# UCL/gp_emulator

Hardware: NVIDIA B200
Metric: test-point predictions/sec (mean+var+grad, M=250, D=10, FP64) (higher is better)
Workload: dtype f64

## Files before the change

gp_emulator_b200/csrc/gpemu.cu:

```cuda
#include <cuda_runtime.h>
#include <pthread.h>
#include <sched.h>
#include <stdarg.h>
#include <stdint.h>
#include <stdio.h>
#include <stdlib.h>
#include <string.h>

#include <algorithm>
#include <atomic>
#include <chrono>
#include <condition_variable>
#include <deque>
#include <cmath>
#include <mutex>
#include <string>
#include <thread>
#include <vector>

#include "../../include/gpemu.h"
#include "launch.h"
#include "predict_generic.cuh"
#include "gpe_math.cuh"
#include "host_common.h"
#include "host_stream.h"
#include "invert.h"

using namespace gpe;

namespace {

thread_local char g_err[512] = "";
std::atomic<int64_t> g_launches{0};
long long* g_trace = nullptr;

int fail(int code, const char* fmt, ...) {
    va_list ap;
    va_start(ap, fmt);
    vsnprintf(g_err, sizeof(g_err), fmt, ap);
    va_end(ap);
    return code;
}

#define CUDA_TRY(expr)                                                                                   \
    do {                                                                                                 \
        cudaError_t _e = (expr);                                                                         \
        if (_e != cudaSuccess)                                                                           \
            return fail(GPE_ERR_CUDA, "%s failed: %s (%s:%d)", #expr, cudaGetErrorString(_e), __FILE__, __LINE__); \
    } while (0)

constexpr uint32_t kSmemMax = 232448;
inline uint32_t align_up(uint32_t x, uint32_t a) { return (x + a - 1) / a * a; }

constexpr int kHessFusedMaxDp = 16;

struct FullPlan {
    bool valid = false;
    int cfg = 0, TN = 0, WC = 0, GH = 1, ctas_per_sm = 1;
    int Mp = 0, nt_act = 0, kblk = 0, kbps = 0, nit = 0, nstage = 0, JC = 0, nchunks = 0;
    uint32_t off_bar = 0, off_sqw = 0, off_ks = 0, off_bst = 0, off_xc = 0, off_ts = 0, off_pa = 0, off_vred = 0;
    uint32_t stage_bytes = 0, smem = 0, ts_bytes = 0;
    uint32_t off_hts = 0;
    int NC = 0, kbh = 0, nit_h = 0;
};

struct Tf32Plan {
    bool valid = false;
    int DP = 0, Mp = 0, nslab = 0;
    bool big = false;
    int pass_cols = 0;
    uint32_t off_bar = 0, off_tmem = 0, off_a = 0, off_b = 0, off_x = 0, off_out = 0, off_vred = 0, bstage_bytes = 0, smem = 0;
};

struct MeanPlan {
    int JC = 0, nchunks = 0;
    uint32_t off_xc = 0, off_ts = 0, off_out = 0, smem = 0, smem_hess = 0;
};

struct BankMeanPlan {
    bool valid = false;
    int G = 0, ngroups = 0, JC = 0, nchunks = 0;
    uint32_t off_x = 0, off_a = 0, off_w = 0, off_ts = 0, smem = 0;
};

}

struct gpe_model {
    int device = 0, M = 0, D = 0, DP = 0, sms = 0;
    const DpKernels* kern = nullptr;
    double b = 0;
    double sqrt_w[32];
    bool has_invQ = false;
    bool symmetric = false;
    FullPlan full;
    FullPlan full_small;
    MeanPlan mean;
    double* d_xchunks_full = nullptr;
    double* d_stiled = nullptr;
    double* d_ptiled = nullptr;
    bool large_valid = false;
    int large_Mp = 0, large_kblk = 0, large_nstage = 0;
    int64_t large_chunk = 0;
    double* d_kscratch = nullptr;
    cudaEvent_t scratch_free = nullptr;
    std::mutex scratch_mu;
    double centre[32];
    bool hess_fused_ok = false;
    double* d_xchunks_mean = nullptr;
    bool generic = false;
    double* d_gen_xs = nullptr;
    double* d_gen_alpha = nullptr;
    double* d_gen_sqw = nullptr;
    double* d_gen_mu = nullptr;
    Tf32Plan tf, tfx;
    float* d_xa_f32 = nullptr;
    uint32_t* d_bslabs = nullptr;
    uint32_t* d_bslabs_lo = nullptr;
    std::vector<double> h_inputs, h_invQt, h_invQ;
    double h_expx[33];
    std::mutex host_mu;
    Slot slots[3];
};

struct gpe_bank {
    int device = 0, E = 0, M = 0, D = 0, W = 0;
    std::vector<gpe_model*> models;
    MeanBankEntry* d_entries = nullptr;
    BankMeanPlan gplan[2];
    double* d_gx = nullptr;
    double* d_galpha[2] = {nullptr, nullptr};
    double* d_gw[2] = {nullptr, nullptr};
    double* d_basis = nullptr;
    int Wp = 0;
    std::mutex host_mu;
    Slot slots[3];
    double* d_aux = nullptr;
    size_t aux_cap = 0;
    cudaEvent_t aux_ready = nullptr;
    std::mutex cost_mu;
    double* cost_d = nullptr;
    size_t cost_cap = 0;
    cudaEvent_t cost_free = nullptr;
    std::mutex solve_mu;
    void* solve_d = nullptr;
    size_t solve_cap = 0;
    int* solve_count = nullptr;
    cudaEvent_t solve_ev = nullptr;
};

struct gpe_multi {
    std::vector<int> devices;
    std::vector<gpe_model*> models;
    std::vector<gpe_bank*> banks;
    std::mutex route_mu;
    bool routed = false;
    std::vector<Relay> relays;
    std::vector<double> link_gbs;
};

namespace {

BankMeanPlan plan_bank_mean(int E, int M, int D, int DP, bool grad) {
    BankMeanPlan g;
    long best = (long)E * (3 * D + 13);
    const int per_em = grad ? 2 * D + 12 : D + 11;
    for (int G = 2; G <= 10; ++G) {
        if (!bank_group_ok(DP, G, grad)) continue;
        const long cost = (long)((E + G - 1) / G) * (G * per_em + 2 * D);
        if (cost < best) { best = cost; g.G = G; }
    }
    if (const char* e = getenv(grad ? "GPE_BANK_G" : "GPE_BANK_G_MEAN"))
        if (bank_group_ok(DP, atoi(e), grad)) g.G = atoi(e);
    if (g.G == 0) return g;
    const int GP = (g.G + 1) & ~1;
    g.ngroups = (E + g.G - 1) / g.G;
    const int m4 = (M + 3) / 4 * 4;
    g.JC = std::min(m4, 256);
    g.nchunks = (M + g.JC - 1) / g.JC;
    uint32_t off = 0;
    g.off_x = off; off += align_up((uint32_t)g.JC * x_pitch(DP) * 8u, 16);
    g.off_a = off; off += align_up((uint32_t)g.JC * GP * 8u, 16);
    g.off_w = off; off += align_up(2u * g.G * DP * 8u, 16);
    g.off_ts = off; off += align_up((uint32_t)kBankTN * (uint32_t)std::max(D, g.G * (grad ? DP + 1 : 1)) * 8u, 16);
    g.smem = off;
    g.valid = true;
    return g;
}

FullPlan plan_full(int M, int D, int DP, int small_Mp = 0) {
    FullPlan f;
    const int m32 = (M + 31) / 32 * 32, m64 = (M + 63) / 64 * 64;
    const uint32_t smem_cap = kSmemMax - 2048;
    if (small_Mp > 0) {
        f.cfg = 2; f.TN = 16; f.WC = 8; f.GH = 4; f.Mp = small_Mp; f.nt_act = small_Mp / 64;
    } else if (m32 <= 256) {
        f.cfg = 0; f.TN = 64; f.WC = 4; f.GH = 1; f.Mp = m32; f.nt_act = m32 / 32;
    } else if (m64 <= 512) {
        f.cfg = 1; f.TN = 32; f.WC = 8; f.GH = 2; f.Mp = m64; f.nt_act = m64 / 64;
    } else if (m64 <= 1024) {
        f.cfg = 2; f.TN = 16; f.WC = 8; f.GH = 4; f.Mp = m64; f.nt_act = m64 / 64;
    } else {
        return f;
    }
    f.ctas_per_sm = 1;
    f.kblk = (M + 3) / 4;
    f.kbps = (f.cfg == 0) ? 2 : 1;
    f.nit = (f.kblk + f.kbps - 1) / f.kbps;
    f.stage_bytes = (uint32_t)f.kbps * f.Mp * 32u;

    uint32_t off = 0;
    f.off_bar = off; off += 192;
    f.off_sqw = off; off += 256;
    f.off_ks = off; off += (uint32_t)f.TN * (f.Mp + 4) * 8u;
    f.ts_bytes = align_up((uint32_t)f.TN * (D + 1) * 8u, 16);
    f.off_ts = off; off += 2 * f.ts_bytes;
    f.off_pa = off; off += (f.GH > 1) ? align_up((uint32_t)f.GH * f.TN * (D + 1) * 8u, 16) : 0;
    f.off_vred = off; off += (uint32_t)f.WC * f.TN * 8u;
    if (DP <= kHessFusedMaxDp) {
        f.off_hts = off; off += align_up((uint32_t)f.TN * D * 8u, 16);
        f.NC = (DP * (DP + 1) / 2 + 7) / 8 * 8;
        f.kbh = (int)(f.stage_bytes / ((uint32_t)f.NC * 32u));
        f.nit_h = f.kbh > 0 ? (f.kblk + f.kbh - 1) / f.kbh : 0;
    }
    off = align_up(off, 128);
    const uint32_t fixed = off;
    const int m4 = (M + 3) / 4 * 4;
    const uint32_t row = (uint32_t)(x_pitch(DP) + 1) * 8u;
    {
        const uint32_t avail = smem_cap - fixed;
        const uint32_t resident = (uint32_t)m4 * row;
        if (avail >= resident + 3 * f.stage_bytes) {
            f.JC = m4; f.nchunks = 1;
        } else {
            if (avail < 2 * f.stage_bytes + 64 * row) return f;
            const int jc_max = (int)((avail - 2 * f.stage_bytes) / row) / 4 * 4;
            f.JC = std::min(std::min(jc_max, 256), m4); f.nchunks = (M + f.JC - 1) / f.JC;
        }
        f.nstage = (int)std::min<uint32_t>(8, (avail - (uint32_t)f.JC * row) / f.stage_bytes);
        if (f.nstage < 2) return f;
    }
    f.off_bst = fixed;
    f.off_xc = fixed + (uint32_t)f.nstage * f.stage_bytes;
    f.smem = f.off_xc + (uint32_t)f.JC * row;
    f.valid = f.smem <= smem_cap;
    return f;
}

MeanPlan plan_mean(int M, int D, int DP) {
    MeanPlan m;
    const int m4 = (M + 3) / 4 * 4;
    m.JC = std::min(m4, 256);
    m.nchunks = (M + m.JC - 1) / m.JC;
    uint32_t off = 0;
    m.off_xc = off; off += align_up((uint32_t)m.JC * (x_pitch(DP) + 1) * 8u, 16);
    m.off_ts = off; off += align_up((uint32_t)kMeanTN * (D + 1) * 8u, 16);
    m.off_out = off;
    m.smem = off;
    m.smem_hess = off + (uint32_t)kMeanTN * D * 8u * (uint32_t)(DP <= 12 ? D : (DP <= 16 ? 4 : 2));
    return m;
}

uint32_t mean_extent(const MeanPlan& mp, int D, int DP, bool hess) {
    uint32_t ext = std::max(mp.off_xc + (uint32_t)mp.JC * (x_pitch(DP) + 1) * 8u, mp.off_ts + (uint32_t)kMeanTN * (D + 1) * 8u);
    if (hess) ext = std::max(ext, mp.off_out + (uint32_t)kMeanTN * D * 8u * (uint32_t)(DP <= 12 ? D : (DP <= 16 ? 4 : 2)));
    return ext;
}

template <typename T>
cudaError_t upload(T** d, const std::vector<T>& h) {
    const cudaError_t e = cudaMalloc((void**)d, h.size() * sizeof(T));
    return e == cudaSuccess ? cudaMemcpy(*d, h.data(), h.size() * sizeof(T), cudaMemcpyHostToDevice) : e;
}

std::vector<double> pack_xchunks(int M, int D, int DP, int JC, int nchunks, const double* inputs,
                                 const double* sqrt_w, const double* invQt, double b) {
    const int XP = x_pitch(DP);
    std::vector<double> buf((size_t)nchunks * JC * (XP + 1), 0.0);
    for (int j = 0; j < M; ++j) {
        const int c = j / JC, jl = j - c * JC;
        double* base = buf.data() + (size_t)c * JC * (XP + 1);
        for (int d = 0; d < D; ++d) base[(size_t)jl * XP + d] = sqrt_w[d] * inputs[(size_t)j * D + d];
        base[(size_t)JC * XP + jl] = b * invQt[j];
    }
    return buf;
}

int check_device(int device, int* sms) {
    int n = 0;
    cudaError_t e = cudaGetDeviceCount(&n);
    if (e != cudaSuccess || n == 0)
        return fail(GPE_ERR_NO_DEVICE, "no CUDA device available (%s); libgpemu has no CPU fallback",
                    e == cudaSuccess ? "device count 0" : cudaGetErrorString(e));
    if (device < 0 || device >= n) return fail(GPE_ERR_INVALID, "device %d out of range [0, %d)", device, n);
    cudaDeviceProp prop;
    CUDA_TRY(cudaGetDeviceProperties(&prop, device));
    if (prop.major != 10)
        return fail(GPE_ERR_NO_DEVICE, "device %d is sm_%d%d; libgpemu kernels are built for sm_100a only", device,
                    prop.major, prop.minor);
    *sms = prop.multiProcessorCount;
    return GPE_OK;
}

constexpr double kHessFusedMaxR2 = 2000.0;

cudaError_t build_hessian_operand(gpe_model* m, const double* inputs, const double* invQt) {
    const FullPlan& f = m->full;
    const int M = m->M, D = m->D;
    memset(m->centre, 0, sizeof(m->centre));
    m->hess_fused_ok = false;
    if (getenv("GPE_HESS_DIRECT") != nullptr) return cudaSuccess;
    if (!f.valid || f.kbh < 1 || f.NC > M || f.NC > f.Mp) return cudaSuccess;
    double r2max = 0.0;
    for (int d = 0; d < D; ++d) {
        double lo = inputs[d], hi = inputs[d];
        for (int j = 1; j < M; ++j) { lo = std::min(lo, inputs[(size_t)j * D + d]); hi = std::max(hi, inputs[(size_t)j * D + d]); }
        m->centre[d] = m->sqrt_w[d] * 0.5 * (lo + hi);
        const double r = m->sqrt_w[d] * 0.5 * (hi - lo);
        r2max = std::max(r2max, r * r);
    }
    if (!(r2max <= kHessFusedMaxR2)) return cudaSuccess;
    std::vector<double> pt((size_t)f.kblk * f.NC * 4, 0.0);
    std::vector<double> xp(D);
    for (int j = 0; j < M; ++j) {
        for (int d = 0; d < D; ++d) xp[d] = m->sqrt_w[d] * inputs[(size_t)j * D + d] - m->centre[d];
        const double ba = m->b * invQt[j];
        int col = 0;
        for (int d = 0; d < D; ++d)
            for (int e = d; e < D; ++e, ++col) pt[((size_t)(j >> 2) * f.NC + col) * 4 + (j & 3)] = ba * xp[d] * xp[e];
    }
    const cudaError_t e = upload(&m->d_ptiled, pt);
    m->hess_fused_ok = e == cudaSuccess;
    return e;
}

cudaError_t setup_large(gpe_model* m, const double* invQ) {
    const int M = m->M;
    m->large_Mp = (M + 63) / 64 * 64;
    m->large_kblk = m->large_Mp / 4;
    m->large_nstage = 6;
    m->large_chunk = 16 * (int64_t)m->sms * 4;
    const size_t scratch = (size_t)(m->large_chunk / 16) * m->large_kblk * 64 * 8;
    cudaError_t e = cudaMalloc((void**)&m->d_kscratch, scratch);
    if (e == cudaSuccess) e = cudaMemset(m->d_kscratch, 0, scratch);
    if (e == cudaSuccess) e = cudaEventCreateWithFlags(&m->scratch_free, cudaEventDisableTiming);
    if (e != cudaSuccess || !invQ || M > GPE_MAX_TRAIN) return e;
    const size_t Mp = (size_t)m->large_Mp;
    std::vector<double> st((size_t)m->large_kblk * Mp * 4, 0.0);
    for (int j = 0; j < M; ++j)
        for (int i = 0; i < M; ++i) st[((size_t)(i >> 2) * Mp + j) * 4 + (i & 3)] = invQ[(size_t)j * M + i];
    e = upload(&m->d_stiled, st);
    m->large_valid = e == cudaSuccess;
    return e;
}

cudaError_t var_large(const gpe_model* m, double* var, int64_t ld_var, int64_t n, cudaStream_t st) {
    VarLargeParams v;
    memset(&v, 0, sizeof(v));
    v.kstar = m->d_kscratch; v.s_tiled = m->d_stiled; v.var = var; v.ld_var = ld_var; v.N = n;
    v.Mp = m->large_Mp; v.kblk = m->large_kblk; v.npass = (m->large_Mp + kVlPass - 1) / kVlPass;
    v.nstage = m->large_nstage; v.b = m->b;
    const size_t smem = 128 + kVlWarps * kVlTN * 8 + (size_t)v.nstage * kVlStageBytes;
    return launch_var_large(v, (int)std::min<int64_t>((n + kVlTN - 1) / kVlTN, m->sms), smem, st);
}

int predict_generic(gpe_model* m, const double* testing, int64_t N, double* mu, double* var, double* deriv, double* hess,
                    int64_t ld_mu, int64_t ld_var, int64_t ld_deriv, int64_t ld_hess, cudaStream_t st) {
    if (var != nullptr && !m->has_invQ) return fail(GPE_ERR_INVALID, "variance requested but the model was created without invQ");
    if (var != nullptr && !m->large_valid)
        return fail(GPE_ERR_UNSUPPORTED, "variance contraction supports M <= %d (got M = %d)", GPE_MAX_TRAIN, m->M);
    const int D = m->D;
    const size_t smem_k = ((size_t)(kGenTN + kGenJC) * (D + 1) + 128) * 8;
    std::lock_guard<std::mutex> scratch_lock(m->scratch_mu);
    CUDA_TRY(cudaStreamWaitEvent(st, m->scratch_free, 0));
    for (int64_t n0 = 0; n0 < N; n0 += m->large_chunk) {
        const int64_t n = std::min(m->large_chunk, N - n0);
        GenericParams p;
        memset(&p, 0, sizeof(p));
        p.testing = testing + n0 * D; p.N = n;
        p.mu = mu ? mu + n0 * ld_mu : nullptr;
        p.deriv = deriv ? deriv + n0 * ld_deriv : nullptr;
        p.hess = hess ? hess + n0 * ld_hess : nullptr;
        p.ld_mu = ld_mu; p.ld_deriv = ld_deriv; p.ld_hess = ld_hess;
        p.xs = m->d_gen_xs; p.alpha = m->d_gen_alpha; p.sqw = m->d_gen_sqw;
        p.kstar = m->d_kscratch; p.mu_tmp = m->d_gen_mu;
        p.M = m->M; p.D = D; p.kblk = m->large_kblk;
        const int64_t tiles = (n + kGenTN - 1) / kGenTN;
        CUDA_TRY(launch_kernel(k_generic_kstar, (unsigned)std::min<int64_t>(tiles, (int64_t)m->sms * 4), kGenThreads, smem_k, st, p));
        if (deriv != nullptr)
            CUDA_TRY(launch_kernel(k_generic_grad, dim3((unsigned)std::min<int64_t>(tiles, (int64_t)m->sms * 8), (unsigned)std::min((D + 15) / 16, 16)),
                                   kGenThreads, 0, st, p));
        if (var != nullptr) CUDA_TRY(var_large(m, var + n0 * ld_var, ld_var, n, st));
        if (hess != nullptr) CUDA_TRY(launch_kernel(k_generic_hess, (unsigned)std::min<int64_t>(n, (int64_t)m->sms * 8), kGenThreads, 0, st, p));
    }
    CUDA_TRY(cudaEventRecord(m->scratch_free, st));
    return GPE_OK;
}

enum class Path { generic, large, tiny, fused, mean };
struct CallPlan {
    Path path;
    const FullPlan* full = nullptr;
    bool fuse_hess = false;
};

CallPlan plan_call(const gpe_model* m, int64_t call_N, bool var, bool hess) {
    CallPlan c;
    if (m->generic) { c.path = Path::generic; return c; }
    static const bool no_tiny = getenv("GPE_NO_TINY") != nullptr;
    static const int64_t env_max = getenv("GPE_TINY_MAX") ? atoll(getenv("GPE_TINY_MAX")) : -1;
    const int64_t tiny_max = env_max >= 0 ? env_max : kTinyTN * (int64_t)(2 * m->sms / kTinyCluster);
    const FullPlan& f = m->full;
    const bool tiny = m->has_invQ && !no_tiny && f.valid && f.cfg == 0 && f.nchunks == 1 && m->DP <= 16 && call_N <= tiny_max;
    c.path = tiny ? Path::tiny : f.valid ? Path::fused : m->large_valid ? Path::large : Path::mean;
    c.fuse_hess = hess && m->hess_fused_ok && !tiny && (var ? !m->symmetric : f.cfg == 0);
    const bool small = m->full_small.valid && !c.fuse_hess && call_N <= 3 * 16 * (int64_t)m->sms;
    c.full = small ? &m->full_small : &m->full;
    return c;
}

int predict_device(gpe_model* m, const double* testing, int64_t N, double* mu, double* var, double* deriv,
                   double* hess, int64_t ld_mu, int64_t ld_var, int64_t ld_deriv, int64_t ld_hess,
                   cudaStream_t st, int64_t call_N = -1) {
    if (call_N < 0) call_N = N;
    if (N == 0) return GPE_OK;
    const CallPlan c = plan_call(m, call_N, var != nullptr, hess != nullptr);
    if (c.path == Path::generic) return predict_generic(m, testing, N, mu, var, deriv, hess, ld_mu, ld_var, ld_deriv, ld_hess, st);
    bool mean_done = false;
    static const bool force_full = getenv("GPE_FORCE_FULL") != nullptr;
    if (var != nullptr && c.path == Path::large) {
        std::lock_guard<std::mutex> scratch_lock(m->scratch_mu);
        CUDA_TRY(cudaStreamWaitEvent(st, m->scratch_free, 0));
        for (int64_t n0 = 0; n0 < N; n0 += m->large_chunk) {
            const int64_t n = std::min(m->large_chunk, N - n0);
            MeanParams p;
            memset(&p, 0, sizeof(p));
            p.testing = testing + n0 * m->D; p.N = n;
            p.mu = mu ? mu + n0 * ld_mu : nullptr;
            p.deriv = deriv ? deriv + n0 * ld_deriv : nullptr;
            p.ld_mu = ld_mu; p.ld_deriv = ld_deriv;
            p.xchunks = m->d_xchunks_mean; p.M = m->M; p.D = m->D; p.JC = m->mean.JC; p.nchunks = m->mean.nchunks;
            p.off_xc = m->mean.off_xc; p.off_ts = m->mean.off_ts; p.off_out = m->mean.off_out;
            p.smem_need = mean_extent(m->mean, m->D, m->DP, false);
            p.kstar = m->d_kscratch; p.kblk = m->large_kblk;
            memcpy(p.sqrt_w, m->sqrt_w, sizeof(p.sqrt_w));
            const int64_t mtiles = (n + kMeanTN - 1) / kMeanTN;
            CUDA_TRY(m->kern->mean(false, p, dim3((unsigned)std::min<int64_t>(mtiles, (int64_t)m->sms * 12)), m->mean.smem, st));
            CUDA_TRY(var_large(m, var + n0 * ld_var, ld_var, n, st));
        }
        CUDA_TRY(cudaEventRecord(m->scratch_free, st));
        mean_done = true;
        var = nullptr;
    }
    if (var != nullptr && c.path == Path::tiny) {
        const FullPlan& f = m->full;
        TinyParams p;
        memset(&p, 0, sizeof(p));
        p.testing = testing; p.N = N; p.mu = mu; p.var = var; p.deriv = deriv;
        p.ld_mu = ld_mu; p.ld_var = ld_var; p.ld_deriv = ld_deriv;
        p.xchunks = m->d_xchunks_full; p.s_tiled = m->d_stiled;
        p.M = m->M; p.D = m->D; p.JC = f.JC; p.Mp = f.Mp; p.kblk = f.kblk; p.b = m->b;
        memcpy(p.sqrt_w, m->sqrt_w, sizeof(p.sqrt_w));
        const size_t work = std::max<size_t>({(size_t)f.JC * (x_pitch(m->DP) + 1) + (size_t)kTinyTN * m->D,
                                              (size_t)16 * 16 * (m->DP + 1), (size_t)8 * 16 * 32});
        const size_t smem = ((size_t)kTinyTN * (f.Mp + 4) + work) * 8;
        const int grid = (int)((N + kTinyTN - 1) / kTinyTN) * kTinyCluster;
        CUDA_TRY(m->kern->tiny(p, grid, smem, st));
        mean_done = true;
        var = nullptr;
    }
    if (var != nullptr || c.fuse_hess || (force_full && m->full.valid)) {
        if (var != nullptr && !m->has_invQ) return fail(GPE_ERR_INVALID, "variance requested but the model was created without invQ");
        if (!m->full.valid)
            return fail(GPE_ERR_UNSUPPORTED, "variance contraction supports M <= %d (got M = %d)", GPE_MAX_TRAIN, m->M);
        const FullPlan& f = *c.full;
        FullParams p;
        memset(&p, 0, sizeof(p));
        p.testing = testing; p.N = N; p.mu = mu; p.var = var; p.deriv = deriv;
        p.ld_mu = ld_mu; p.ld_var = ld_var; p.ld_deriv = ld_deriv;
        p.xchunks = m->d_xchunks_full; p.s_tiled = m->d_stiled;
        p.M = m->M; p.D = m->D; p.Mp = f.Mp; p.nt_act = f.nt_act; p.kblk = f.kblk;
        p.nit = f.nit; p.nstage = f.nstage; p.lag = (f.nstage >= 3) ? 2 : 1; p.symmetric = (m->symmetric && var != nullptr) ? 1 : 0;
        if (const char* e = getenv("GPE_RING_LAG")) p.lag = std::max(1, std::min(atoi(e), f.nstage - 1));
        p.skew = (f.cfg == 0 && f.nt_act == 8) ? 300 : 0;
        if (const char* e = getenv("GPE_SKEW")) p.skew = atoi(e);
        p.JC = f.JC; p.nchunks = f.nchunks; p.b = m->b;
        p.off_bar = f.off_bar; p.off_sqw = f.off_sqw; p.off_ks = f.off_ks; p.off_bst = f.off_bst;
        p.off_xc = f.off_xc; p.off_ts = f.off_ts; p.off_pa = f.off_pa; p.off_vred = f.off_vred;
        p.stage_bytes = f.stage_bytes; p.ts_bytes = f.ts_bytes;
        memcpy(p.sqrt_w, m->sqrt_w, sizeof(p.sqrt_w));
        p.trace = g_trace;
        if (c.fuse_hess) {
            p.hess = hess; p.ld_hess = ld_hess; p.p_tiled = m->d_ptiled; p.kbh = f.kbh; p.nit_h = f.nit_h; p.off_hts = f.off_hts;
            memcpy(p.centre, m->centre, sizeof(p.centre));
            hess = nullptr;
        }
        const int64_t ntiles = (N + f.TN - 1) / f.TN;
        const int grid = (int)std::min<int64_t>(ntiles, (int64_t)m->sms * f.ctas_per_sm);
        CUDA_TRY(m->kern->full(f.cfg, p, grid, f.smem, st));
        mean_done = true;
    }
    const bool need_mean = !mean_done && (mu != nullptr || deriv != nullptr);
    if (need_mean || hess != nullptr) {
        const bool do_hess = hess != nullptr;
        MeanParams p;
        memset(&p, 0, sizeof(p));
        p.testing = testing; p.N = N;
        p.mu = mean_done ? nullptr : mu;
        p.deriv = mean_done ? nullptr : deriv;
        p.hess = hess;
        p.ld_mu = ld_mu; p.ld_deriv = ld_deriv; p.ld_hess = ld_hess;
        p.xchunks = m->d_xchunks_mean; p.M = m->M; p.D = m->D; p.JC = m->mean.JC; p.nchunks = m->mean.nchunks;
        p.off_xc = m->mean.off_xc; p.off_ts = m->mean.off_ts; p.off_out = m->mean.off_out;
        p.smem_need = mean_extent(m->mean, m->D, m->DP, do_hess);
        memcpy(p.sqrt_w, m->sqrt_w, sizeof(p.sqrt_w));
        const int64_t ntiles = (N + kMeanTN - 1) / kMeanTN;
        static const int env_mult = getenv("GPE_MEAN_GRID") ? atoi(getenv("GPE_MEAN_GRID")) : 0;
        const int mult = env_mult > 0 ? env_mult : (do_hess ? 8 : 12);
        const int grid = (int)std::min<int64_t>(ntiles, (int64_t)m->sms * mult);
        const size_t smem = do_hess ? m->mean.smem_hess : m->mean.smem;
        CUDA_TRY(m->kern->mean(do_hess, p, dim3(grid), smem, st));
    }
    return GPE_OK;
}

struct DeviceRestore {
    int dev = -1;
    DeviceRestore() { if (cudaGetDevice(&dev) != cudaSuccess) { cudaGetLastError(); dev = -1; } }
    ~DeviceRestore() { if (dev >= 0) cudaSetDevice(dev); }
};

struct IoList {
    IoSpec v[kMaxIo];
    int n = 0;
    int add(const void* host, int64_t width) {
        if (n >= kMaxIo) return -1;
        v[n].host = const_cast<void*>(host);
        v[n].width = width;
        return n++;
    }
};

void bind_thread_near_device(int device) {
    char bdf[32];
    if (cudaDeviceGetPCIBusId(bdf, sizeof(bdf), device) != cudaSuccess) { cudaGetLastError(); return; }
    for (char* c = bdf; *c; ++c) *c = (char)tolower(*c);
    const std::string path = std::string("/sys/bus/pci/devices/") + bdf + "/local_cpulist";
    FILE* f = fopen(path.c_str(), "r");
    if (!f) return;
    char line[4096];
    cpu_set_t set;
    CPU_ZERO(&set);
    int count = 0;
    if (fgets(line, sizeof(line), f)) {
        char* save = nullptr;
        for (char* tok = strtok_r(line, ",\n", &save); tok; tok = strtok_r(nullptr, ",\n", &save)) {
            int a = 0, b = 0;
            if (sscanf(tok, "%d-%d", &a, &b) == 2) { for (int i = a; i <= b && i < CPU_SETSIZE; ++i) { CPU_SET(i, &set); ++count; } }
            else if (sscanf(tok, "%d", &a) == 1 && a < CPU_SETSIZE) { CPU_SET(a, &set); ++count; }
        }
    }
    fclose(f);
    if (count > 0) pthread_setaffinity_np(pthread_self(), sizeof(set), &set);
}

template <typename Fn>
int run_per_device(int G, const int* devices, Fn fn) {
    std::vector<int> rcs(G, GPE_OK);
    std::vector<std::string> msgs(G);
    std::vector<std::thread> th;
    for (int g = 0; g < G; ++g)
        th.emplace_back([&, g] {
            bind_thread_near_device(devices[g]);
            if (cudaSetDevice(devices[g]) != cudaSuccess) rcs[g] = fail(GPE_ERR_CUDA, "cudaSetDevice(%d) failed", devices[g]);
            else rcs[g] = fn(g);
            if (rcs[g]) msgs[g] = gpe_last_error();
        });
    for (auto& t : th) t.join();
    for (int g = 0; g < G; ++g)
        if (rcs[g]) return fail(rcs[g], "device %d: %s", devices[g], msgs[g].c_str());
    return GPE_OK;
}

template <typename... T>
int take_outputs(unsigned flags, T*&... outs) {
    unsigned bit = GPE_WANT_MU;
    bool missing = false, any = false;
    auto take = [&](auto*& o) {
        if (!(flags & bit)) o = nullptr;
        else if (!o) missing = true;
        any = any || o != nullptr;
        bit <<= 1;
    };
    (take(outs), ...);
    if (missing) return fail(GPE_ERR_INVALID, "an output flag is set but its array is NULL");
    if (!any) return fail(GPE_ERR_INVALID, "no output requested");
    return GPE_OK;
}

struct CallIo {
    IoList in, out;
    int idx[6] = {-1, -1, -1, -1, -1, -1};
    template <typename T>
    T* at(void* const* chunk, int k) const { return idx[k] >= 0 ? (T*)chunk[idx[k]] : nullptr; }
};

CallIo model_io(int64_t D, const void* testing, const void* mu, const void* var, const void* deriv, const void* hess) {
    CallIo io;
    io.in.add(testing, D);
    io.idx[0] = mu ? io.out.add(mu, 1) : -1;
    io.idx[1] = var ? io.out.add(var, 1) : -1;
    io.idx[2] = deriv ? io.out.add(deriv, D) : -1;
    io.idx[3] = hess ? io.out.add(hess, D * D) : -1;
    return io;
}

struct SharedCall {
    const StreamPlan* plan;
    ChunkSource* src;
    const Relay* relay;
};

StreamPlan stream_plan(const CallIo& io, int64_t N, size_t ES, int sms, int shared_by = 0) {
    return plan_stream(io.in.v, io.in.n, io.out.v, io.out.n, N, ES, 64 * (int64_t)sms, std::max(shared_by, 1), shared_by == 0);
}

template <typename Launch>
int stream_call(Slot* slots, int device, int sms, const CallIo& io, int64_t N, size_t ES, const SharedCall* shared,
                Launch launch) {
    const StreamPlan pl = shared ? *shared->plan : stream_plan(io, N, ES, sms);
    int rc = prepare_slots(slots, pl, io.in.v, io.in.n, io.out.v, io.out.n, ES);
    if (rc) return rc;
    std::atomic<int64_t> cursor{0};
    const ChunkSource src = shared ? *shared->src : ChunkSource{&cursor, N, pl.CH};
    return stream_host(slots, device, pl, src, ES, io.in.v, io.in.n, io.out.v, io.out.n, launch, shared ? shared->relay : nullptr);
// ... 1421 lines not shown
```

gp_emulator_b200/csrc/predict_full.cuh:

```cuda
#pragma once
#include <cuda_runtime.h>
#include <stdint.h>
#include <type_traits>
#include "gpe_math.cuh"
#include "gpe_ptx.cuh"

namespace gpe {

constexpr int kMaxD = 32;

struct FullParams {
    const double* testing;
    int64_t N;
    double* mu;
    double* var;
    double* deriv;
    int64_t ld_mu, ld_var, ld_deriv;
    const double* xchunks;
    const double* s_tiled;
    int M, D;
    int Mp;
    int nt_act;
    int kblk;
    int nit;
    int nstage;
    int lag;
    int JC;
    int symmetric;
    int skew;
    int nchunks;
    double b;
    uint32_t off_bar, off_sqw, off_ks, off_bst, off_xc, off_ts, off_pa, off_vred;
    uint32_t ts_bytes;
    uint32_t stage_bytes;
    double* hess;
    int64_t ld_hess;
    const double* p_tiled;
    int kbh;
    int nit_h;
    uint32_t off_hts;
    long long* trace;
    double sqrt_w[kMaxD];
    double centre[kMaxD];
};

template <int I, int N, typename F>
__device__ __forceinline__ void static_for_impl(F& f) {
    if constexpr (I < N) {
        f(std::integral_constant<int, I>{});
        static_for_impl<I + 1, N>(f);
    }
}
template <int N, typename F>
__device__ __forceinline__ void static_for(F f) {
    static_for_impl<0, N>(f);
}

template <int MT, int NT, int WR, int WC, int DP, int MINB, int KB, bool FULLNT, bool SYM, bool HESS>
__global__ void __launch_bounds__(WR * WC * 32, MINB) k_predict_full(const FullParams p) {
    constexpr int NW = WR * WC;
    constexpr int NTHR = NW * 32;
    constexpr int TN = WR * MT * 8;
    constexpr int NHI = TN / 8;
    constexpr int GH = NW / NHI;
    constexpr int TPR = NTHR / TN;
    constexpr int NV = DP + 1;
    constexpr int XP = x_pitch(DP);
    static_assert((NW & (NW - 1)) == 0, "warp count must be a power of two");
    static_assert(NHI * GH == NW && NHI >= 1 && GH >= 1, "TN must be 8 * (a divisor of the warp count)");
    static_assert(TPR >= 1 && TPR * TN == NTHR, "TN must divide the thread count");
    static_assert(DP % 2 == 0, "DP even (16-byte rows)");
    constexpr bool kLateChores = (MT >= 4);
    constexpr int NMT = TN / 8;
    constexpr int CG = (NW >= NMT) ? NW / NMT : 1;
    constexpr int NCT = (DP * (DP + 1) / 2 + 7) / 8;
    constexpr int NC = NCT * 8;
    constexpr int NTH = (NCT + CG - 1) / CG;
    static_assert(!HESS || (NW % NMT == 0 && NW >= NMT), "phase C needs the row tiles to divide the warps");
    static_assert(!(HESS && SYM), "the fused Hessian is built for the plain variance operand only");

    extern __shared__ __align__(128) unsigned char smem[];
    uint64_t* bar_full = reinterpret_cast<uint64_t*>(smem + p.off_bar);
    uint64_t* bar_empty = bar_full + 8;
    uint64_t* bar_x = bar_full + 16;
    uint64_t* bar_t = bar_full + 17;
    double* sqw_s = reinterpret_cast<double*>(smem + p.off_sqw);
    double* Ks = reinterpret_cast<double*>(smem + p.off_ks);
    unsigned char* Bst = smem + p.off_bst;
    double* Xc = reinterpret_cast<double*>(smem + p.off_xc);
    double* pa_s = reinterpret_cast<double*>(smem + p.off_pa);
    double* vred = reinterpret_cast<double*>(smem + p.off_vred);
    double* hts = reinterpret_cast<double*>(smem + p.off_hts);
    __shared__ int htab[HESS ? 256 : 1];
    __shared__ double cen_s[HESS ? kMaxD : 1];
    __shared__ double exp_tab[64];

    const int tid = threadIdx.x, warp = tid >> 5, lane = tid & 31;
    const int D = p.D, M = p.M, Mp = p.Mp;
    const int pitch = Mp + 4;
    const int nstage = p.nstage;
    const int lag = p.lag;
    const int DV = D + 1;

    const int64_t ntiles = (p.N + TN - 1) / TN;
    const bool want_var = (p.var != nullptr);
    const bool want_hess = HESS && (p.hess != nullptr);
    const int nit_b = want_var ? p.nit : 0;
    const int nit_tot = nit_b + (want_hess ? p.nit_h : 0);
    const bool ts_tma_ok = (reinterpret_cast<uintptr_t>(p.testing) & 15) == 0;
    const uint32_t ts_tile_bytes = (uint32_t)TN * D * 8u;

    {
        uint32_t ext = umax2(p.off_bar + 192u, p.off_sqw + 256u);
        ext = umax2(ext, p.off_ks + (uint32_t)TN * (uint32_t)pitch * 8u);
        ext = umax2(ext, p.off_ts + 2u * p.ts_bytes);
        ext = umax2(ext, umax2((uint32_t)TN * (uint32_t)DV * 8u, ts_tile_bytes) + p.off_ts + p.ts_bytes);
        if (GH > 1) ext = umax2(ext, p.off_pa + (uint32_t)GH * TN * (uint32_t)DV * 8u);
        ext = umax2(ext, p.off_vred + (uint32_t)WC * TN * 8u);
        if (want_hess) ext = umax2(ext, p.off_hts + (uint32_t)TN * (uint32_t)D * 8u);
        if (nit_tot > 0) ext = umax2(ext, p.off_bst + (uint32_t)nstage * p.stage_bytes);
        ext = umax2(ext, p.off_xc + (uint32_t)p.JC * (XP + 1) * 8u);
        smem_guard(ext);
    }
    if (tid == 0) {
        for (int s = 0; s < nstage; ++s) {
            mbar_init(&bar_full[s], 1);
            mbar_init(&bar_empty[s], NW);
        }
        mbar_init(bar_x, 1);
        mbar_init(&bar_t[0], 1);
        mbar_init(&bar_t[1], 1);
        fence_mbar_init();
    }
    if (tid < kMaxD) sqw_s[tid] = p.sqrt_w[tid];
    exp_tab_load(exp_tab, tid);
    if (HESS) {
        if (tid < kMaxD) cen_s[tid] = p.centre[tid];
        for (int e = tid; e < p.D * p.D; e += NTHR) {
            const int d1 = e / p.D, d2 = e - d1 * p.D;
            const int lo = min(d1, d2), hi = max(d1, d2);
            htab[e] = d1 | (d2 << 8) | ((lo * p.D - lo * (lo - 1) / 2 + hi - lo) << 16);
        }
    }
    for (int r = warp; r < TN; r += NW)
        for (int c = M + lane; c < pitch; c += 32) Ks[r * pitch + c] = 0.0;
    __syncthreads();

    int cs = 0;
    uint32_t cpar = 0;
    auto issue = [&](int stage, int it_local) {
        if (HESS && it_local >= nit_b) {
            const int kb0 = (it_local - nit_b) * p.kbh;
            const uint32_t bytes = (uint32_t)min(p.kbh, p.kblk - kb0) * (uint32_t)NC * 32u;
            mbar_arrive_expect_tx(&bar_full[stage], bytes);
            tma_bulk_g2s(Bst + (size_t)stage * p.stage_bytes, p.p_tiled + (size_t)kb0 * NC * 4, bytes, &bar_full[stage]);
            return;
        }
        const int kb0 = it_local * KB;
        const int nkb = min(KB, p.kblk - kb0);
        unsigned char* dst = Bst + (size_t)stage * p.stage_bytes;
        if (!SYM) {
            const uint32_t bytes = (uint32_t)nkb * (uint32_t)Mp * 32u;
            mbar_arrive_expect_tx(&bar_full[stage], bytes);
            tma_bulk_g2s(dst, p.s_tiled + (size_t)kb0 * Mp * 4, bytes, &bar_full[stage]);
        } else {
            uint32_t total = 0;
            for (int kk = 0; kk < nkb; ++kk) total += (uint32_t)(Mp - 8 * ((kb0 + kk) >> 1)) * 32u;
            mbar_arrive_expect_tx(&bar_full[stage], total);
            for (int kk = 0; kk < nkb; ++kk) {
                const int c0 = 8 * ((kb0 + kk) >> 1);
                tma_bulk_g2s(dst + ((size_t)kk * Mp + c0) * 32, p.s_tiled + ((size_t)(kb0 + kk) * Mp + c0) * 4,
                             (uint32_t)(Mp - c0) * 32u, &bar_full[stage]);
            }
        }
    };
    auto issue_burst = [&]() {
        const int burst = min(nstage, nit_tot);
        if (lane == 0) {
            for (int i = warp; i < burst; i += NW) {
                int s = cs + i;
                if (s >= nstage) s -= nstage;
                issue(s, i);
            }
        }
    };
    auto refill = [&](int it) {
        if (it >= lag && lane == 0 && warp == (it & (NW - 1)) && it - lag + nstage < nit_tot) {
            const int ps = (cs >= lag) ? cs - lag : cs - lag + nstage;
            const uint32_t ppar = (cs >= lag) ? cpar : (cpar ^ 1);
            mbar_wait(&bar_empty[ps], ppar);
            issue(ps, it - lag + nstage);
        }
    };
    uint32_t xpar = 0;
    bool x_resident = false;

    uint32_t tpar = 0;
    auto prefetch_rows = [&](int64_t tile, int buf) -> bool {
        const int64_t n0 = tile * TN;
        if (!ts_tma_ok || n0 + TN > p.N) return false;
        fence_proxy_async();
        mbar_arrive_expect_tx(&bar_t[buf], ts_tile_bytes);
        tma_bulk_g2s(smem + p.off_ts + (size_t)buf * p.ts_bytes, p.testing + n0 * D, ts_tile_bytes, &bar_t[buf]);
        return true;
    };
    auto rows_prefetched = [&](int64_t tile) { return ts_tma_ok && (tile * TN + TN <= p.N); };

    const int g_low = lane & 7, n_low = lane >> 3;
    const int n_hi = warp % NHI, g_hi = warp / NHI;
    const int n_a = n_hi * 8 + n_low, n_b = n_a + 4;
    const int wrow = warp / WC;
    const int wcol = (SYM && ((warp >> 2) & 1)) ? (((warp % WC) & ~3) | (3 - ((warp % WC) & 3))) : warp % WC;
    const int nt_act = FULLNT ? NT : p.nt_act;

    int buf = 0;
    if (tid == 0 && blockIdx.x < ntiles) prefetch_rows(blockIdx.x, 0);
    int trace_tile = 0;
    const bool tracing = p.trace != nullptr && blockIdx.x == 0 && tid == 0;
#define GPE_TRACE(k) do { if (tracing && trace_tile < 64) p.trace[trace_tile * 8 + (k)] = clock64(); } while (0)

    for (int64_t tile = blockIdx.x; tile < ntiles; tile += gridDim.x, buf ^= 1) {
        const int64_t n0 = tile * TN;
        const int npts = (int)min((int64_t)TN, p.N - n0);
        double* ts_s = reinterpret_cast<double*>(smem + p.off_ts + (size_t)buf * p.ts_bytes);
        GPE_TRACE(0);
        if (!kLateChores && nit_tot > 0) issue_burst();

        if (rows_prefetched(tile)) {
            mbar_wait(&bar_t[buf], (tpar >> buf) & 1u);
            tpar ^= 1u << buf;
        } else {
            for (int e = tid; e < TN * D; e += NTHR) {
                const int r = e / D;
                const int64_t src = (r < npts) ? (n0 * D + e) : ((p.N - 1) * D + (e - r * D));
                ts_s[e] = __ldg(p.testing + src);
            }
            __syncthreads();
        }
        constexpr bool kTwoPass = DP > 16;
        double tsa[kTwoPass ? 1 : DP], tsb[kTwoPass ? 1 : DP];
        if constexpr (!kTwoPass) {
#pragma unroll
            for (int d = 0; d < DP; ++d) {
                tsa[d] = (d < D) ? ts_s[n_a * D + d] * sqw_s[d] : 0.0;
                tsb[d] = (d < D) ? ts_s[n_b * D + d] * sqw_s[d] : 0.0;
            }
        }
        if constexpr (HESS) {
            if (want_hess && g_hi == 0) {
#pragma unroll
                for (int d = 0; d < DP; ++d)
                    if ((d & 7) == g_low && d < D) {
                        hts[n_a * D + d] = tsa[d] - cen_s[d];
                        hts[n_b * D + d] = tsb[d] - cen_s[d];
                    }
            }
        }
        if (!x_resident && tid == 0) {
            const uint32_t bytes = (uint32_t)p.JC * (XP + 1) * 8u;
            mbar_arrive_expect_tx(bar_x, bytes);
            tma_bulk_g2s(Xc, p.xchunks, bytes, bar_x);
        }
        __syncthreads();
        if (kLateChores && nit_tot > 0) issue_burst();
        {
            const int64_t next = tile + gridDim.x;
            if (tid == ((kLateChores && NW > 4) ? 32 * (NW - 1) : 0) && next < ntiles) prefetch_rows(next, buf ^ 1);
        }

        GPE_TRACE(1);
        double va[NV], vb[NV];
#pragma unroll
        for (int i = 0; i < NV; ++i) va[i] = vb[i] = 0.0;

        for (int c = 0; c < p.nchunks; ++c) {
            if (!x_resident) {
                if (c > 0 && tid == 0) {
                    const uint32_t bytes = (uint32_t)p.JC * (XP + 1) * 8u;
                    mbar_arrive_expect_tx(bar_x, bytes);
                    tma_bulk_g2s(Xc, p.xchunks + (size_t)c * p.JC * (XP + 1), bytes, bar_x);
                }
                mbar_wait(bar_x, xpar);
                xpar ^= 1;
                if (p.nchunks == 1) x_resident = true;
            }
            const int jn = min(p.JC, M - c * p.JC);
            const double* al = Xc + p.JC * XP;
            double* krow_a = Ks + n_a * pitch + c * p.JC;
            double* krow_b = krow_a + 4 * pitch;
            if constexpr (kTwoPass) {
                auto sweep = [&](int n_r, double (&v1)[NV]) {
                    double* krow = Ks + n_r * pitch + c * p.JC;
                    double ts1[DP];
#pragma unroll
                    for (int d = 0; d < DP; ++d) ts1[d] = (d < D) ? ts_s[n_r * D + d] * sqw_s[d] : 0.0;
                    for (int jl = 8 * g_hi + g_low; jl < jn; jl += 8 * GH) {
                        const double2* xr = reinterpret_cast<const double2*>(Xc + jl * XP);
                        double u[DP];
                        double r = 0.0;
#pragma unroll
                        for (int q = 0; q < DP / 2; ++q) {
                            const double2 x2 = xr[q];
                            u[2 * q] = x2.x - ts1[2 * q];
                            u[2 * q + 1] = x2.y - ts1[2 * q + 1];
                            r = fma(u[2 * q], u[2 * q], r);
                            r = fma(u[2 * q + 1], u[2 * q + 1], r);
                        }
                        const double k = exp_neg_tab(-0.5 * r, exp_tab);
                        krow[jl] = k;
                        const double cj = k * al[jl];
                        v1[0] += cj;
#pragma unroll
                        for (int d = 0; d < DP; ++d) v1[1 + d] = fma(cj, u[d], v1[1 + d]);
                    }
                };
                sweep(n_a, va);
                sweep(n_b, vb);
            } else {
            int jl = 8 * g_hi + g_low;
                if (jl < jn) {
                    double2 xn[DP / 2];
                    double aln;
                    {
                        const double2* xr = reinterpret_cast<const double2*>(Xc + jl * XP);
    #pragma unroll
                        for (int q = 0; q < DP / 2; ++q) xn[q] = xr[q];
                        aln = al[jl];
                    }
                    for (; jl < jn; jl += 8 * GH) {
                        double2 x[DP / 2];
    #pragma unroll
                        for (int q = 0; q < DP / 2; ++q) x[q] = xn[q];
                        const double alj = aln;
                        {
                            const int jnx = min(jl + 8 * GH, jn - 1);
                            const double2* xr = reinterpret_cast<const double2*>(Xc + jnx * XP);
    #pragma unroll
                            for (int q = 0; q < DP / 2; ++q) xn[q] = xr[q];
                            aln = al[jnx];
                        }
                        double ua[DP], ub[DP];
                        double ra = 0.0, rb = 0.0;
    #pragma unroll
                        for (int q = 0; q < DP / 2; ++q) {
                            const int d = 2 * q;
                            ua[d] = x[q].x - tsa[d];
                            ub[d] = x[q].x - tsb[d];
                            ua[d + 1] = x[q].y - tsa[d + 1];
                            ub[d + 1] = x[q].y - tsb[d + 1];
                            ra = fma(ua[d], ua[d], ra);
                            rb = fma(ub[d], ub[d], rb);
                            ra = fma(ua[d + 1], ua[d + 1], ra);
                            rb = fma(ub[d + 1], ub[d + 1], rb);
                        }
                        const double ka = exp_neg_tab(-0.5 * ra, exp_tab);
                        const double kb = exp_neg_tab(-0.5 * rb, exp_tab);
                        krow_a[jl] = ka;
                        krow_b[jl] = kb;
                        const double ca = ka * alj, cb = kb * alj;
                        va[0] += ca;
                        vb[0] += cb;
    #pragma unroll
                        for (int d = 0; d < DP; ++d) {
                            va[1 + d] = fma(ca, ua[d], va[1 + d]);
                            vb[1 + d] = fma(cb, ub[d], vb[1 + d]);
                        }
                    }
                }
            }
            if (!x_resident) __syncthreads();
        }

        GPE_TRACE(2);
        double* outs = ts_s;
        if constexpr (kTwoPass) __syncthreads();
        {
            RS<NV> rs;
            rs.run(va, vb, lane);
            double* dst = ((GH == 1) ? outs : pa_s + g_hi * TN * DV) + ((lane & 4) ? n_b : n_a) * DV;
            const int half_base = (lane & 2) ? RS<NV>::H2 : 0;
            const int base3 = (lane & 1) ? RS<NV>::H3 : 0;
#pragma unroll
            for (int i = 0; i < RS<NV>::H3; ++i) {
                const int i2 = base3 + i;
                const int idx = half_base + i2;
                if (i2 < RS<NV>::H2 && idx < DV) dst[idx] = rs.r3[i];
            }
            __syncthreads();
            if (GH > 1) {
                for (int e = tid; e < TN * DV; e += NTHR) {
                    double sum = 0.0;
                    for (int gh = 0; gh < GH; ++gh) sum += pa_s[gh * TN * DV + e];
                    outs[e] = sum;
                }
                __syncthreads();
            }
        }
        {
            const int r = tid / TPR, q = tid % TPR;
            if (r < npts) {
                if (p.mu != nullptr && q == 0) p.mu[(n0 + r) * p.ld_mu] = outs[r * DV];
                if (p.deriv != nullptr) {
                    for (int d = q; d < D; d += TPR) p.deriv[(n0 + r) * p.ld_deriv + d] = sqw_s[d] * outs[r * DV + 1 + d];
                }
            }
        }

        GPE_TRACE(3);
        if (want_var) {
            double acc[MT][NT][2];
#pragma unroll
            for (int i = 0; i < MT; ++i)
#pragma unroll
                for (int j = 0; j < NT; ++j) acc[i][j][0] = acc[i][j][1] = 0.0;

            const double* a_base = Ks + (wrow * MT * 8 + (lane >> 2)) * pitch + (lane & 3);
            const int b_off = (wcol * 8 + (lane >> 2)) * 4 + (lane & 3);

            auto ring_step = [&](auto jm_c, int it) {
                constexpr int JM = decltype(jm_c)::value;
                refill(it);
                const int kb0 = it * KB;
                double a[KB][MT];
#pragma unroll
                for (int kk = 0; kk < KB; ++kk)
#pragma unroll
                    for (int i = 0; i < MT; ++i) a[kk][i] = a_base[i * 8 * pitch + (kb0 + kk) * 4];
                mbar_wait(&bar_full[cs], cpar);
                const double* bs = reinterpret_cast<const double*>(Bst + (size_t)cs * p.stage_bytes) + b_off;
#pragma unroll
                for (int kk = 0; kk < KB; ++kk) {
                    if (KB == 1 || kb0 + kk < p.kblk) {
                        const double* bk = bs + kk * Mp * 4;
#pragma unroll
                        for (int j = JM; j < NT; ++j) {
                            if (!FULLNT && j >= nt_act) break;
                            const double bf = bk[j * (WC * 32)];
#pragma unroll
                            for (int i = 0; i < MT; ++i) dmma_m8n8k4(acc[i][j][0], acc[i][j][1], a[kk][i], bf);
                        }
                    }
                }
                __syncwarp();
                if (lane == 0) mbar_arrive(&bar_empty[cs]);
                if (++cs == nstage) { cs = 0; cpar ^= 1; }
            };
            if (p.skew > 0 && ((warp >> 2) & 1)) {
                const long long t0 = clock64();
                while (clock64() - t0 < p.skew) {}
            }
            if constexpr (!SYM) {
                for (int it = 0; it < nit_b; ++it) ring_step(std::integral_constant<int, 0>{}, it);
            } else {
                int it = 0;
                static_for<NT>([&](auto jm_c) {
                    constexpr int JM = decltype(jm_c)::value;
                    const int it_end = min(nit_b, (WC * JM + wcol + 1) * (2 / KB));
                    for (; it < it_end; ++it) ring_step(jm_c, it);
                });
                for (; it < nit_b; ++it) ring_step(std::integral_constant<int, NT>{}, it);
            }

            GPE_TRACE(4);
            double vs[MT];
#pragma unroll
            for (int i = 0; i < MT; ++i) vs[i] = 0.0;
            const int odd = (lane >> 2) & 1;
            const double* k_base = Ks + (wrow * MT * 8 + (lane >> 2)) * pitch + wcol * 8 + 2 * (lane & 3);
#pragma unroll
            for (int j = 0; j < NT; ++j) {
                if (FULLNT || j < nt_act) {
#pragma unroll
                    for (int i = 0; i < MT; ++i) {
                        const double* kp = k_base + i * 8 * pitch + j * (WC * 8);
                        if (kLateChores) {
                            const double k_first = kp[odd], k_second = kp[odd ^ 1];
                            vs[i] = fma(acc[i][j][0], odd ? k_second : k_first, vs[i]);
                            vs[i] = fma(acc[i][j][1], odd ? k_first : k_second, vs[i]);
                        } else {
                            const double2 kk = *reinterpret_cast<const double2*>(kp);
                            vs[i] = fma(acc[i][j][0], kk.x, vs[i]);
                            vs[i] = fma(acc[i][j][1], kk.y, vs[i]);
                        }
                    }
                }
            }
#pragma unroll
            for (int i = 0; i < MT; ++i) {
                vs[i] += __shfl_xor_sync(0xffffffffu, vs[i], 1);
                vs[i] += __shfl_xor_sync(0xffffffffu, vs[i], 2);
                if ((lane & 3) == 0) vred[wcol * TN + wrow * MT * 8 + i * 8 + (lane >> 2)] = vs[i];
            }
            __syncthreads();
            if (tid < npts) {
                double v = 0.0;
#pragma unroll
                for (int w = 0; w < WC; ++w) v += vred[w * TN + tid];
                p.var[(n0 + tid) * p.ld_var] = p.b - p.b * p.b * v;
            }
        }
        if (HESS && want_hess) {
            GPE_TRACE(5);
            const int mt = warp % NMT, cg = warp / NMT;
            double hacc[NTH][2];
#pragma unroll
            for (int j = 0; j < NTH; ++j) hacc[j][0] = hacc[j][1] = 0.0;
            const double* a_base = Ks + (mt * 8 + (lane >> 2)) * pitch + (lane & 3);
            const int b_off = (cg * 8 + (lane >> 2)) * 4 + (lane & 3);
            for (int it = nit_b; it < nit_tot; ++it) {
                refill(it);
                const int kb0 = (it - nit_b) * p.kbh;
                const int nkb = min(p.kbh, p.kblk - kb0);
                mbar_wait(&bar_full[cs], cpar);
                const double* bs = reinterpret_cast<const double*>(Bst + (size_t)cs * p.stage_bytes) + b_off;
                const double* ap = a_base + kb0 * 4;
#pragma unroll 3
                for (int kk = 0; kk < nkb; ++kk) {
                    const double a = ap[kk * 4];
                    const double* bk = bs + kk * (NC * 4);
#pragma unroll
                    for (int j = 0; j < NTH; ++j) {
                        if (NCT % CG != 0 && cg + CG * j >= NCT) break;
                        dmma_m8n8k4(hacc[j][0], hacc[j][1], a, bk[j * (CG * 32)]);
                    }
                }
                __syncwarp();
                if (lane == 0) mbar_arrive(&bar_empty[cs]);
                if (++cs == nstage) { cs = 0; cpar ^= 1; }
            }
            GPE_TRACE(6);
            __syncthreads();
#pragma unroll
            for (int j = 0; j < NTH; ++j) {
                if (cg + CG * j < NCT)
                    *reinterpret_cast<double2*>(Ks + (mt * 8 + (lane >> 2)) * pitch + (cg + CG * j) * 8 + 2 * (lane & 3)) =
                        make_double2(hacc[j][0], hacc[j][1]);
            }
            __syncthreads();
            constexpr int NE = (DP * DP + 31) / 32;
            const int DD = D * D;
            int o1[NE], o2[NE], oc[NE];
            double ow[NE], od[NE];
#pragma unroll
            for (int i = 0; i < NE; ++i) {
                const int e = min(lane + 32 * i, DD - 1);
                const int t = htab[e];
                o1[i] = t & 255; o2[i] = (t >> 8) & 255; oc[i] = t >> 16;
                ow[i] = sqw_s[o1[i]] * sqw_s[o2[i]];
                od[i] = (o1[i] == o2[i]) ? ow[i] : 0.0;
            }
#pragma unroll 2
            for (int r = warp; r < npts; r += NW) {
                const double* s2 = Ks + r * pitch;
                const double* tp = hts + r * D;
                const double* g = outs + r * DV + 1;
                const double s0 = outs[r * DV];
                double* dst = p.hess + (n0 + r) * p.ld_hess;
#pragma unroll
                for (int i = 0; i < NE; ++i) {
                    const double t1 = tp[o1[i]], t2 = tp[o2[i]];
                    double v = s2[oc[i]];
                    v = fma(-t1, g[o2[i]], v);
                    v = fma(-t2, fma(t1, s0, g[o1[i]]), v);
                    v = fma(v, ow[i], -od[i] * s0);
                    if (lane + 32 * i < DD) dst[lane + 32 * i] = v;
                }
            }
            GPE_TRACE(7);
        }
        __syncthreads();
        if (!(HESS && want_hess)) GPE_TRACE(5);
        ++trace_tile;
    }
}

#undef GPE_TRACE

}
```

Baseline: 219.4 million.

## Pack multiple triangular k-blocks per ring stage in symmetric variance path

In the symmetric variance path each ring stage used to carry one k-block unit with trailing columns skipped, so stages were partly empty. A host-computed schedule now packs several consecutive shrinking triangular units into one stage buffer. This cuts the number of ring iterations, mbarrier waits and refills. The cost is a per-unit sub-step loop that walks a variable packed offset, plus a 512-byte schedule array added to the kernel parameters.

```diff
diff --git a/gp_emulator_b200/csrc/gpemu.cu b/gp_emulator_b200/csrc/gpemu.cu
--- a/gp_emulator_b200/csrc/gpemu.cu
+++ b/gp_emulator_b200/csrc/gpemu.cu
@@ -62,6 +62,8 @@
     uint32_t stage_bytes = 0, smem = 0, ts_bytes = 0;
     uint32_t off_hts = 0;
     int NC = 0, kbh = 0, nit_h = 0;
+    int sym_nit = 0;
+    uint16_t sym_stage_end[kMaxSymStages];
 };
 
 struct Tf32Plan {
@@ -207,6 +209,7 @@
     f.kbps = (f.cfg == 0) ? 2 : 1;
     f.nit = (f.kblk + f.kbps - 1) / f.kbps;
     f.stage_bytes = (uint32_t)f.kbps * f.Mp * 32u;
+    f.sym_nit = sym_stage_schedule(f.kblk, f.kbps, f.Mp, f.stage_bytes, f.sym_stage_end);
 
     uint32_t off = 0;
     f.off_bar = off; off += 192;
@@ -480,6 +483,10 @@
         p.xchunks = m->d_xchunks_full; p.s_tiled = m->d_stiled;
         p.M = m->M; p.D = m->D; p.Mp = f.Mp; p.nt_act = f.nt_act; p.kblk = f.kblk;
         p.nit = f.nit; p.nstage = f.nstage; p.lag = (f.nstage >= 3) ? 2 : 1; p.symmetric = (m->symmetric && var != nullptr) ? 1 : 0;
+        if (p.symmetric) {
+            p.nit = f.sym_nit;
+            memcpy(p.sym_stage_end, f.sym_stage_end, sizeof(p.sym_stage_end));
+        }
         if (const char* e = getenv("GPE_RING_LAG")) p.lag = std::max(1, std::min(atoi(e), f.nstage - 1));
         p.skew = (f.cfg == 0 && f.nt_act == 8) ? 300 : 0;
         if (const char* e = getenv("GPE_SKEW")) p.skew = atoi(e);
diff --git a/gp_emulator_b200/csrc/predict_full.cuh b/gp_emulator_b200/csrc/predict_full.cuh
--- a/gp_emulator_b200/csrc/predict_full.cuh
+++ b/gp_emulator_b200/csrc/predict_full.cuh
@@ -8,6 +8,7 @@
 namespace gpe {
 
 constexpr int kMaxD = 32;
+constexpr int kMaxSymStages = 256;
 
 struct FullParams {
     const double* testing;
@@ -42,7 +43,25 @@
     long long* trace;
     double sqrt_w[kMaxD];
     double centre[kMaxD];
+    uint16_t sym_stage_end[kMaxSymStages];
 };
+
+__host__ __device__ inline int sym_stage_schedule(int kblk, int KB, int Mp, uint32_t stage_bytes, uint16_t* end) {
+    const int nunits = (kblk + KB - 1) / KB;
+    int nst = 0;
+    uint32_t fill = 0;
+    for (int u = 0; u < nunits; ++u) {
+        uint32_t bytes = 0;
+        for (int kb = u * KB; kb < (u + 1) * KB && kb < kblk; ++kb) bytes += (uint32_t)(Mp - 8 * (kb >> 1)) * 32u;
+        if (u > 0 && fill + bytes > stage_bytes) {
+            end[nst++] = (uint16_t)u;
+            fill = 0;
+        }
+        fill += bytes;
+    }
+    end[nst++] = (uint16_t)nunits;
+    return nst;
+}
 
 template <int I, int N, typename F>
 __device__ __forceinline__ void static_for_impl(F& f) {
@@ -164,13 +183,17 @@
             mbar_arrive_expect_tx(&bar_full[stage], bytes);
             tma_bulk_g2s(dst, p.s_tiled + (size_t)kb0 * Mp * 4, bytes, &bar_full[stage]);
         } else {
-            uint32_t total = 0;
-            for (int kk = 0; kk < nkb; ++kk) total += (uint32_t)(Mp - 8 * ((kb0 + kk) >> 1)) * 32u;
-            mbar_arrive_expect_tx(&bar_full[stage], total);
-            for (int kk = 0; kk < nkb; ++kk) {
-                const int c0 = 8 * ((kb0 + kk) >> 1);
-                tma_bulk_g2s(dst + ((size_t)kk * Mp + c0) * 32, p.s_tiled + ((size_t)(kb0 + kk) * Mp + c0) * 4,
-                             (uint32_t)(Mp - c0) * 32u, &bar_full[stage]);
+            const int kb_lo = (it_local == 0 ? 0 : (int)p.sym_stage_end[it_local - 1]) * KB;
+            const int kb_hi = min((int)p.sym_stage_end[it_local] * KB, p.kblk);
+            auto F = [](int n) { return n > 0 ? (n >> 1) * ((n - 1) >> 1) : 0; };
+            mbar_arrive_expect_tx(&bar_full[stage], (uint32_t)(Mp * (kb_hi - kb_lo) - 8 * (F(kb_hi) - F(kb_lo))) * 32u);
+            uint32_t off = 0;
+#pragma unroll 1
+            for (int kb = kb_lo; kb < kb_hi; ++kb) {
+                const int c0 = 8 * (kb >> 1);
+                const uint32_t bytes = (uint32_t)(Mp - c0) * 32u;
+                tma_bulk_g2s(dst + off, p.s_tiled + ((size_t)kb * Mp + c0) * 4, bytes, &bar_full[stage]);
+                off += bytes;
             }
         }
     };
@@ -452,13 +475,54 @@
             if constexpr (!SYM) {
                 for (int it = 0; it < nit_b; ++it) ring_step(std::integral_constant<int, 0>{}, it);
             } else {
-                int it = 0;
+                const int nunits = (p.kblk + KB - 1) / KB;
+                int st = 0, st_lo = 0, st_hi = p.sym_stage_end[0];
+                int boff = 0;
+                auto sub_step = [&](auto jm_c, int u) {
+                    constexpr int JM = decltype(jm_c)::value;
+                    const bool first = (u == st_lo);
+                    if (first) refill(st);
+                    const int kb0 = u * KB;
+                    double a[KB][MT];
+#pragma unroll
+                    for (int kk = 0; kk < KB; ++kk)
+#pragma unroll
+                        for (int i = 0; i < MT; ++i) a[kk][i] = a_base[i * 8 * pitch + (kb0 + kk) * 4];
+                    if (first) mbar_wait(&bar_full[cs], cpar);
+                    const double* bs = reinterpret_cast<const double*>(Bst + (size_t)cs * p.stage_bytes) + b_off;
+#pragma unroll
+                    for (int kk = 0; kk < KB; ++kk) {
+                        if (KB == 1 || kb0 + kk < p.kblk) {
+                            const int c0 = 8 * ((kb0 + kk) >> 1);
+                            const double* bk = bs + (boff - c0 * 4);
+                            boff += (Mp - c0) * 4;
+#pragma unroll
+                            for (int j = JM; j < NT; ++j) {
+                                if (!FULLNT && j >= nt_act) break;
+                                const double bf = bk[j * (WC * 32)];
+#pragma unroll
+                                for (int i = 0; i < MT; ++i) dmma_m8n8k4(acc[i][j][0], acc[i][j][1], a[kk][i], bf);
+                            }
+                        }
+                    }
+                    if (u + 1 == st_hi) {
+                        __syncwarp();
+                        if (lane == 0) mbar_arrive(&bar_empty[cs]);
+                        if (++cs == nstage) { cs = 0; cpar ^= 1; }
+                        if (++st < nit_b) {
+                            st_lo = st_hi;
+                            st_hi = p.sym_stage_end[st];
+                        }
+                        boff = 0;
+                    }
+                };
+                int u = 0;
                 static_for<NT>([&](auto jm_c) {
                     constexpr int JM = decltype(jm_c)::value;
-                    const int it_end = min(nit_b, (WC * JM + wcol + 1) * (2 / KB));
-                    for (; it < it_end; ++it) ring_step(jm_c, it);
+                    const int u_end = min(nunits, (WC * JM + wcol + 1) * (2 / KB));
+                    for (; u < u_end; ++u) sub_step(jm_c, u);
                 });
-                for (; it < nit_b; ++it) ring_step(std::integral_constant<int, NT>{}, it);
+                for (; u < nunits; ++u) sub_step(std::integral_constant<int, NT>{}, u);
             }
 
             GPE_TRACE(4);
```

Measured after the change: 219.4 million, median of 6. No clear change (+0.0%).
